# wmtlab/tactileSR

Hardware: AMD Instinct MI355X
Metric: SR samples/sec (4x4->40x40) (higher is better)
Workload: dtype f32 as 2 power-of-two-scaled fp16 planes x 3 MFMA products, fp32 accumulate (fp32-grade); 1 GPU; tactileSR_model eval forward 4x4->40x40, batch=4096/GPU, fp32 in/out (BASELINE configs[1]); batch_per_gpu=4096, scale_factor=10, seqsCnt=1, parallelism=replicas x1, conv_impl=fp16x3, dist_world_size=1

## Files before the change

### tactilesr_amd/csrc/conv_epilogue16.h

```cpp
#pragma once
#include "tsr_common.h"
#include "conv_args.h"
#include "conv_epilogue.h"

template <int COUT, bool EXT, int WN = 2, bool IO16 = false>
__device__ __forceinline__ void conv_epilogue16(const ConvArgs& a, f32x4 (&acc)[4][COUT / (16 * WN)], int ebase, int b0,
                                                int y0, int x0, int wm, int wn, int lane, int HW, float accmul = 1.f) {
  constexpr int NT = COUT / (16 * WN);
  const int cl = lane & 15, ph = lane >> 4;
  const int k4 = cl >> 2, j = cl & 3;
  const int dyl = ph >> 1, dxl = 4 * (ph & 1);
  float amax = 0.f;
  const int b = b0 + wm;
  const bool img_ok = b < a.B;
  const int out_blocks = a.out_ctot >> 4;
  const int res_blocks = a.res_ctot >> 4;
  const int mask_blocks = a.mask_ctot >> 4;
  const int bsafe = img_ok ? b : 0;
  typedef __bf16 ep_bf16x4 __attribute__((ext_vector_type(4)));
  const int gx = x0 + dxl + j;
  const f32x4 one4v = {1.f, 1.f, 1.f, 1.f}, zero4v = {0.f, 0.f, 0.f, 0.f};
  f32x4 pv0[NT], pv1[NT], pv2[NT], pv3[NT], pv4[NT];
  const bool m2 = EXT && a.epi_mode == 2, m0 = !EXT || a.epi_mode == 0;
#pragma unroll
  for (int nt = 0; nt < NT; ++nt) {
    const int nq = wn * (COUT / WN) + nt * 16 + 4 * k4;
    pv0[nt] = one4v; pv1[nt] = zero4v; pv2[nt] = one4v; pv3[nt] = zero4v; pv4[nt] = zero4v;
    if (m0) {
      if (a.scale) pv0[nt] = *(const f32x4*)(a.scale + nq);
      if (a.shift) pv1[nt] = *(const f32x4*)(a.shift + nq);
      if (EXT && a.res_scale) { pv2[nt] = *(const f32x4*)(a.res_scale + nq); pv3[nt] = *(const f32x4*)(a.res_shift + nq); }
    } else if (m2) {
      if (a.scale) pv0[nt] = *(const f32x4*)(a.scale + nq);
      if (a.mask_scale) { pv2[nt] = *(const f32x4*)(a.mask_scale + nq); pv1[nt] = *(const f32x4*)(a.mask_shift + nq); }
      if (a.bn_a) { pv3[nt] = *(const f32x4*)(a.bn_a + nq); pv4[nt] = *(const f32x4*)(a.bn_b + nq); }
    }
  }
#pragma unroll
  for (int nt = 0; nt < NT; ++nt) {
    const int n = wn * (COUT / WN) + nt * 16 + cl;
    const int nq = wn * (COUT / WN) + nt * 16 + 4 * k4;
    const int oq = a.out_coff + nq;
    const size_t oidx4 = (((size_t)bsafe * out_blocks + (oq >> 4)) * HW) * 16 + (oq & 15);
    float* ob4 = a.out + oidx4;
    const float* rb4 = nullptr;
    size_t ridx4 = 0;
    if (a.res) {
      const int rq = a.res_coff + nq;
      ridx4 = (((size_t)bsafe * res_blocks + (rq >> 4)) * HW) * 16 + (rq & 15);
      rb4 = a.res + ridx4;
    }
    if (!EXT || a.epi_mode == 0) {
      const f32x4 sc4 = pv0[nt], sh4 = pv1[nt], rsc4 = pv2[nt], rsh4 = pv3[nt];
      f32x4 rvv[4];
#pragma unroll
      for (int mt = 0; mt < 4; ++mt) {
        const int gy = y0 + 2 * mt + dyl;
        const unsigned pr = (img_ok && gy < a.H && gx < a.W) ? (unsigned)(gy * a.W + gx) * 16u : 0u;
        rvv[mt] = (f32x4){0.f, 0.f, 0.f, 0.f};
        if (rb4) {
          if (IO16) {
            const ep_bf16x4 r16 = *(const ep_bf16x4*)((const __bf16*)a.res + ridx4 + pr);
#pragma unroll
            for (int c = 0; c < 4; ++c) rvv[mt][c] = (float)r16[c];
          } else {
            rvv[mt] = *(const f32x4*)(rb4 + pr);
          }
        }
      }
#pragma unroll
      for (int mt = 0; mt < 4; ++mt) {
        float t0 = acc[mt][nt][0], t1 = acc[mt][nt][1], t2 = acc[mt][nt][2], t3 = acc[mt][nt][3];
        quad_transpose(t0, t1, t2, t3, j);
        const int gy = y0 + 2 * mt + dyl;
        if (img_ok && gy < a.H && gx < a.W) {
          const size_t po = (size_t)(gy * a.W + gx) * 16;
          f32x4 v = {t0, t1, t2, t3};
#pragma unroll
          for (int c = 0; c < 4; ++c) v[c] = (v[c] * accmul) * sc4[c] + sh4[c];
          if (rb4) {
            f32x4 rv = rvv[mt];
            if (EXT && a.res_scale) {
#pragma unroll
              for (int c = 0; c < 4; ++c) rv[c] = tsr_relu(fmaf(rv[c], rsc4[c], rsh4[c]));
            }
#pragma unroll
            for (int c = 0; c < 4; ++c) v[c] += rv[c];
          }
#pragma unroll
          for (int c = 0; c < 4; ++c) {
            if (a.relu) v[c] = tsr_relu(v[c]);
            amax = fmaxf(amax, fabsf(v[c]));
          }
          if (IO16) {
            ep_bf16x4 o16;
#pragma unroll
            for (int c = 0; c < 4; ++c) o16[c] = (__bf16)v[c];
            *(ep_bf16x4*)((__bf16*)a.out + oidx4 + po) = o16;
          } else {
            *(f32x4*)(ob4 + po) = v;
          }
        }
      }
    } else if (EXT && a.epi_mode == 1) {
      float cnt = 0.f, sum = 0.f;
#pragma unroll
      for (int mt = 0; mt < 4; ++mt) {
#pragma unroll
        for (int r = 0; r < 4; ++r) {
          const int gy = y0 + 2 * mt + dyl, gxr = x0 + dxl + r;
          acc[mt][nt][r] *= accmul;
          if (img_ok && gy < a.H && gxr < a.W) {
            const float v = acc[mt][nt][r];
            cnt += 1.f;
            sum += v;
            amax = fmaxf(amax, fabsf(v));
          }
        }
      }
      float mean = cnt > 0.f ? sum / cnt : 0.f;
      float m2 = 0.f;
#pragma unroll
      for (int mt = 0; mt < 4; ++mt) {
#pragma unroll
        for (int r = 0; r < 4; ++r) {
          const int gy = y0 + 2 * mt + dyl, gxr = x0 + dxl + r;
          if (img_ok && gy < a.H && gxr < a.W) {
            const float d = acc[mt][nt][r] - mean;
            m2 = fmaf(d, d, m2);
          }
        }
      }
#pragma unroll
      for (int o = 16; o <= 32; o <<= 1) {
        const float cnt2 = __shfl_xor(cnt, o), mean2 = __shfl_xor(mean, o), m22 = __shfl_xor(m2, o);
        const float tot = cnt + cnt2;
        const float dlt = mean2 - mean;
        const float meanm = tot > 0.f ? mean + dlt * (cnt2 / tot) : 0.f;
        const float m2m = tot > 0.f ? m2 + m22 + dlt * dlt * (cnt * cnt2 / tot) : 0.f;
        cnt = tot; mean = meanm; m2 = m2m;
      }
      if (ph == 0) {
        const size_t e = (size_t)ebase + wm;
        float* sl = a.slab + (e * COUT + n) * 2;
        sl[0] = mean;
        sl[1] = m2;
        if (nt == 0 && cl == 0 && wn == 0) a.slab_cnt[e] = cnt;
      }
#pragma unroll
      for (int mt = 0; mt < 4; ++mt) {
        float t0 = acc[mt][nt][0], t1 = acc[mt][nt][1], t2 = acc[mt][nt][2], t3 = acc[mt][nt][3];
        quad_transpose(t0, t1, t2, t3, j);
        const int gy = y0 + 2 * mt + dyl;
        if (img_ok && gy < a.H && gx < a.W) *(f32x4*)(ob4 + (size_t)(gy * a.W + gx) * 16) = (f32x4){t0, t1, t2, t3};
      }
    } else if (EXT) {
      const int mq = a.mask_coff + nq;
      const float* mb4 = a.mask + (((size_t)bsafe * mask_blocks + (mq >> 4)) * HW) * 16 + (mq & 15);
      const f32x4 zero4 = zero4v;
      const f32x4 sc4 = pv0[nt], msc4 = pv2[nt], msh4 = pv1[nt], ba4 = pv3[nt], bb4 = pv4[nt];
      f32x4 s1 = zero4, s2 = zero4;
      f32x4 mvv[4], rvv[4];
      bool okk[4];
      unsigned pov[4];
#pragma unroll
      for (int mt = 0; mt < 4; ++mt) {
        const int gy = y0 + 2 * mt + dyl;
        okk[mt] = img_ok && gy < a.H && gx < a.W;
        pov[mt] = okk[mt] ? (unsigned)(gy * a.W + gx) * 16u : 0u;
        mvv[mt] = *(const f32x4*)(mb4 + pov[mt]);
        rvv[mt] = rb4 ? *(const f32x4*)(rb4 + pov[mt]) : zero4;
      }
#pragma unroll
      for (int mt = 0; mt < 4; ++mt) {
        float t0 = acc[mt][nt][0], t1 = acc[mt][nt][1], t2 = acc[mt][nt][2], t3 = acc[mt][nt][3];
        quad_transpose(t0, t1, t2, t3, j);
        f32x4 v = {t0, t1, t2, t3};
        const f32x4 mv = okk[mt] ? mvv[mt] : zero4, rv = rvv[mt];
#pragma unroll
        for (int c = 0; c < 4; ++c) {
          float x = (v[c] * accmul) * sc4[c] + rv[c];
          if (!(fmaf(mv[c], msc4[c], msh4[c]) > 0.f)) x = 0.f;
          if (!okk[mt]) x = 0.f;
          v[c] = x;
          amax = fmaxf(amax, fabsf(x));
          s1[c] += x;
// ... 28 lines not shown
```

### tactilesr_amd/csrc/conv_fuse1x1_16.h

```cpp
#pragma once
#include "tsr_common.h"
#include "conv_args.h"
#include "conv_epilogue.h"

typedef _Float16 fq_f16x8 __attribute__((ext_vector_type(8)));
typedef _Float16 fq_f16x4 __attribute__((ext_vector_type(4)));

template <int IMG> struct Fuse1x1Geom16 {
  static constexpr int PIXB = 64;
  static constexpr int ROWB = (8 * 4 + 2) * 16;
  static constexpr int IMGB = 8 * ROWB;
  static constexpr int BLKB = IMG * IMGB;
  static constexpr int BYTES = 8 * BLKB;
};

template <int IMG>
__device__ __forceinline__ void conv_fuse1x1_epilogue16(const ConvArgs& a, f32x4 (&acc)[4][4], char* lds, int b0, int y0,
                                                        int x0, int wm, int wn, int lane, int HW, float accmul) {
  typedef Fuse1x1Geom16<IMG> E;
  const int cl = lane & 15, ph = lane >> 4;
  const int k4 = cl >> 2, j = cl & 3;
  const int dyl = ph >> 1, dxl = 4 * (ph & 1);
  const int b = b0 + wm;
  const bool img_ok = b < a.B;
  const int khalf = ph & 1, bsel = ph >> 1;
  const _Float16* wb = (const _Float16*)a.w2 + ((size_t)(bsel * 2 * 2 + khalf) * 64 + wn * 32 + cl) * 8;
  fq_f16x8 fb[4][2][2];
#pragma unroll
  for (int kk = 0; kk < 4; ++kk)
#pragma unroll
    for (int p = 0; p < 2; ++p)
#pragma unroll
      for (int n2 = 0; n2 < 2; ++n2)
        fb[kk][p][n2] = *(const fq_f16x8*)(wb + (size_t)((2 * kk) * 2 + p) * (2 * 64 * 8) + n2 * 16 * 8);
  const int out_blocks = a.out_ctot >> 4, res_blocks = a.res_ctot >> 4;
  const int bsafe = img_ok ? b : 0;
  const int gx = x0 + dxl + j;
  bool okk[4];
  unsigned pov[4];
  f32x4 rvv[2][4];
#pragma unroll
  for (int mt = 0; mt < 4; ++mt) {
    const int gy = y0 + 2 * mt + dyl;
    okk[mt] = img_ok && gy < a.H && gx < a.W;
    pov[mt] = okk[mt] ? (unsigned)(gy * a.W + gx) * 16u : 0u;
  }
#pragma unroll
  for (int n2 = 0; n2 < 2; ++n2) {
    const int rq = a.res_coff + wn * 32 + n2 * 16 + 4 * k4;
    const float* rb4 = a.res ? a.res + (((size_t)bsafe * res_blocks + (rq >> 4)) * HW) * 16 + (rq & 15) : nullptr;
#pragma unroll
    for (int mt = 0; mt < 4; ++mt) rvv[n2][mt] = rb4 ? *(const f32x4*)(rb4 + pov[mt]) : (f32x4){0.f, 0.f, 0.f, 0.f};
  }
  float bsc[4], bsh[4];
  f32x4 osh[2];
#pragma unroll
  for (int nt = 0; nt < 4; ++nt) {
    const int n = wn * 64 + nt * 16 + cl;
    bsc[nt] = a.scale ? a.scale[n] : 1.f;
    bsh[nt] = a.shift ? a.shift[n] : 0.f;
  }
#pragma unroll
  for (int n2 = 0; n2 < 2; ++n2)
    osh[n2] = a.shift2 ? *(const f32x4*)(a.shift2 + wn * 32 + n2 * 16 + 4 * k4) : (f32x4){0.f, 0.f, 0.f, 0.f};
  float amax = 0.f;
#pragma unroll
  for (int nt = 0; nt < 4; ++nt) {
    const float sc = bsc[nt] * accmul, sh = bsh[nt];
#pragma unroll
    for (int mt = 0; mt < 4; ++mt)
#pragma unroll
      for (int r = 0; r < 4; ++r) {
        const int gy = y0 + 2 * mt + dyl, gx = x0 + dxl + r;
        float v = fmaf(acc[mt][nt][r], sc, sh);
        if (a.relu) v = tsr_relu(v);
        if (!(img_ok && gy < a.H && gx < a.W)) v = 0.f;
        acc[mt][nt][r] = v;
        amax = fmaxf(amax, fabsf(v));
      }
  }
#pragma unroll
  for (int o = 32; o > 0; o >>= 1) amax = fmaxf(amax, __shfl_xor(amax, o));
  float* red = (float*)(lds + E::BYTES);
  if (lane == 0) red[wm * 2 + wn] = amax;
  __syncthreads();
  float tmax = 0.f;
#pragma unroll
  for (int w = 0; w < 2 * IMG; ++w) tmax = fmaxf(tmax, red[w] < 3.0e38f ? red[w] : 0.f);
  float s_e = 1.f;
  if (tmax > 0.f) {
    int e = (int)((__float_as_uint(tmax) >> 23) & 0xFF) - 127;
    int be = 13 - e + 127;
    be = be < 1 ? 1 : (be > 254 ? 254 : be);
    s_e = __uint_as_float((unsigned)be << 23);
  }
#pragma unroll
  for (int nt = 0; nt < 4; ++nt) {
    const int nq = wn * 64 + nt * 16 + 4 * k4;
    char* eb = lds + (nq >> 4) * E::BLKB + wm * E::IMGB + dyl * E::ROWB + (dxl + j) * E::PIXB + (nq & 15) * 2;
#pragma unroll
    for (int mt = 0; mt < 4; ++mt) {
      float t0 = acc[mt][nt][0], t1 = acc[mt][nt][1], t2 = acc[mt][nt][2], t3 = acc[mt][nt][3];
      quad_transpose(t0, t1, t2, t3, j);
      float v[4] = {t0 * s_e, t1 * s_e, t2 * s_e, t3 * s_e};
      fq_f16x4 p0, p1;
#pragma unroll
      for (int c = 0; c < 4; ++c) {
        p0[c] = (_Float16)v[c];
        p1[c] = (_Float16)(v[c] - (float)p0[c]);
      }
      char* dst = eb + (2 * mt) * E::ROWB;
      *(fq_f16x4*)(dst) = p0;
      *(fq_f16x4*)(dst + 32) = p1;
    }
  }
  __syncthreads();
  f32x4 acc2[4][2];
#pragma unroll
  for (int mt = 0; mt < 4; ++mt)
#pragma unroll
    for (int n2 = 0; n2 < 2; ++n2) acc2[mt][n2] = (f32x4){0.f, 0.f, 0.f, 0.f};
  const char* ea = lds + bsel * E::BLKB + wm * E::IMGB + (cl >> 3) * E::ROWB + (cl & 7) * E::PIXB + khalf * 16;
#pragma unroll
  for (int kk = 0; kk < 4; ++kk) {
    fq_f16x8 fa[2][4];
#pragma unroll
    for (int p = 0; p < 2; ++p) {
#pragma unroll
      for (int mt = 0; mt < 4; ++mt) fa[p][mt] = *(const fq_f16x8*)(ea + (2 * kk) * E::BLKB + (2 * mt) * E::ROWB + p * 32);
    }
#pragma unroll
    for (int mt = 0; mt < 4; ++mt)
#pragma unroll
      for (int n2 = 0; n2 < 2; ++n2)
        acc2[mt][n2] = __builtin_amdgcn_mfma_f32_16x16x32_f16(fa[1][mt], fb[kk][0][n2], acc2[mt][n2], 0, 0, 0);
#pragma unroll
    for (int mt = 0; mt < 4; ++mt)
#pragma unroll
      for (int n2 = 0; n2 < 2; ++n2)
        acc2[mt][n2] = __builtin_amdgcn_mfma_f32_16x16x32_f16(fa[0][mt], fb[kk][1][n2], acc2[mt][n2], 0, 0, 0);
#pragma unroll
    for (int mt = 0; mt < 4; ++mt)
#pragma unroll
      for (int n2 = 0; n2 < 2; ++n2)
        acc2[mt][n2] = __builtin_amdgcn_mfma_f32_16x16x32_f16(fa[0][mt], fb[kk][0][n2], acc2[mt][n2], 0, 0, 0);
  }
  const float mul2 = a.w2_inv_scale / s_e;
  float omax = 0.f;
#pragma unroll
  for (int n2 = 0; n2 < 2; ++n2) {
    const int nq2 = wn * 32 + n2 * 16 + 4 * k4;
    const int oq = a.out_coff + nq2;
    const f32x4 sh4 = osh[n2];
    float* ob4 = a.out + (((size_t)bsafe * out_blocks + (oq >> 4)) * HW) * 16 + (oq & 15);
#pragma unroll
    for (int mt = 0; mt < 4; ++mt) {
      float t0 = acc2[mt][n2][0], t1 = acc2[mt][n2][1], t2 = acc2[mt][n2][2], t3 = acc2[mt][n2][3];
      quad_transpose(t0, t1, t2, t3, j);
      if (okk[mt]) {
        f32x4 v = {t0, t1, t2, t3};
        const f32x4 rv = rvv[n2][mt];
#pragma unroll
        for (int c = 0; c < 4; ++c) {
          v[c] = v[c] * mul2 + sh4[c] + rv[c];
          if (a.relu2) v[c] = tsr_relu(v[c]);
          omax = fmaxf(omax, fabsf(v[c]));
        }
        *(f32x4*)(ob4 + pov[mt]) = v;
      }
    }
  }
  if (a.out_amax) {
#pragma unroll
    for (int o = 32; o > 0; o >>= 1) omax = fmaxf(omax, __shfl_xor(omax, o));
    if (lane == 0) publish_amax(a.out_amax, omax);
  }
}
```

### tactilesr_amd/csrc/conv_mfma_k32.hip

```cpp
#include "tsr_common.h"
#include "conv_args.h"
#include "conv_epilogue16.h"
#include "conv_fuse1x1_16.h"
#include "conv_host.h"
#include "tactilesr_hip.h"
#include <type_traits>

typedef _Float16 kf16x8 __attribute__((ext_vector_type(8)));
typedef _Float16 kf16x4 __attribute__((ext_vector_type(4)));

constexpr int k32_row_slots(int px) {
  int rs = px * 4;
  while ((rs & 3) != 2) ++rs;
  return rs;
}

template <int KS, int COUT, int WN, bool DBH = false, int NTHR = 256> struct K32Geom {
  static constexpr int IMG = (NTHR / 64) / WN;
  static constexpr int HH = 8 + KS - 1;
  static constexpr int T = KS * KS;
  static constexpr int HS = (T - 1) / 2;
  static constexpr int PIXB = 64;
  static constexpr int ROWB = k32_row_slots(HH) * 16;
  static constexpr int IMGB = HH * ROWB;
  static constexpr int HALO_B = IMG * IMGB;
  static constexpr int SROWB = k32_row_slots(8) * 16;
  static constexpr int SIMGB = 8 * SROWB;
  static constexpr int SIDE_B = DBH ? 0 : IMG * SIMGB;
  static constexpr int WTAP_B = 2 * 16 * COUT * 2;
  static constexpr int WSLAB_B = 2 * WTAP_B;
  static constexpr int NHB = DBH ? 2 : 1;
  static constexpr int MAIN_LDS = NHB * HALO_B + SIDE_B + 3 * WSLAB_B;
};

constexpr int PAIR_KH[12] = {0, 0, 0, 2, 1, 3, 4, 4, 1, 1, 2, 3};
constexpr int PAIR_KW[12] = {0, 2, 4, 4, 0, 0, 1, 3, 1, 3, 1, 1};
constexpr int PAIR_V[12] = {0, 0, 1, 1, 1, 1, 0, 0, 0, 1, 0, 0};
constexpr int PAIR_OUTER = 8;

template <int KS, int COUT, bool EXT, int WN, bool FUSE2 = false, bool DBH = false, int NTHR = 256, bool PAIR = false>
__global__ __launch_bounds__(NTHR, NTHR == 512 ? 1 : 2) void conv_k32_kernel(const ConvArgs a) {
  static_assert(!PAIR || (KS == 5 && COUT == 128 && !EXT && !FUSE2 && !DBH), "pair form: 5x5 geometry, inference");
  static_assert(COUT == 64 * WN, "every wave owns 64 channels");
  static_assert(!FUSE2 || (!EXT && COUT == 128), "fused 1x1: 128 channels, inference");
  static_assert(NTHR == 256 || (NTHR == 512 && WN == 2), "512 threads: 4 images x 2 C_out halves");
  typedef K32Geom<KS, COUT, WN, DBH, NTHR> G;
  constexpr int NW = NTHR / 64;
  constexpr bool WDMA = !EXT;
  constexpr int IMG = G::IMG, P = KS / 2, HH = G::HH, T = G::T, HS = G::HS, NT = COUT / (16 * WN);
  constexpr int PIXB = G::PIXB, ROWB = G::ROWB, IMGB = G::IMGB, HALO_B = G::HALO_B;
  constexpr int SROWB = G::SROWB, SIMGB = G::SIMGB, SIDE_B = G::SIDE_B;
  constexpr int WTAP_B = G::WTAP_B, WSLAB_B = G::WSLAB_B;
  constexpr int WITEMS = WSLAB_B / 16, WV = (WITEMS + NTHR - 1) / NTHR;
  constexpr int NITEM = IMG * HH * HH * 4, NIT = (NITEM + NTHR - 1) / NTHR;
  constexpr int FUSE_LDS = FUSE2 ? Fuse1x1Geom16<IMG>::BYTES + 64 : 0;
  __shared__ __attribute__((aligned(16))) char lds[G::MAIN_LDS > FUSE_LDS ? G::MAIN_LDS : FUSE_LDS];
  char* halo = lds;
  char* wbuf = lds + G::NHB * HALO_B + SIDE_B;

  const int tid = threadIdx.x;
  const int lane = tid & 63;
  const int wave = tid >> 6;
  const int wave_s = __builtin_amdgcn_readfirstlane(wave);
  const int wm = WN == 2 ? wave >> 1 : wave, wn = WN == 2 ? wave & 1 : 0;
  const int m = lane & 15, g = lane >> 4, khalf = g & 1, tsel = g >> 1;

  float sx = 1.f, accmul = 1.f, sxh = 1.f;
  int bid;
  {
    const int nwg = gridDim.x, q = nwg >> 3, r = nwg & 7;
    const int xcd = blockIdx.x & 7, idx = blockIdx.x >> 3;
    bid = (xcd < r ? xcd * (q + 1) : r * (q + 1) + (xcd - r) * q) + idx;
  }
  const int tpi = a.tiles_x * a.tiles_y;
  const int ig = bid / tpi;
  const int trem = bid - ig * tpi;
  const int ebase = bid * IMG;
  const int ty = trem / a.tiles_x, tx = trem - ty * a.tiles_x;
  const int y0 = ty * 8, x0 = tx * 8, b0 = ig * IMG;
  const int HW = a.H * a.W;
  const int in_blocks = a.in_ctot >> 4;

  int st_src[NIT], st_dst[NIT];
#pragma unroll
  for (int k = 0; k < NIT; ++k) {
    const int it = tid + k * NTHR;
    st_src[k] = -1;
    st_dst[k] = -1;
    if (it < NITEM) {
      const int qd = it & 3, px = it >> 2;
      const int img = px / (HH * HH), rem = px - img * (HH * HH);
      const int hy = rem / HH, hx = rem - hy * HH;
      const int gy = y0 - P + hy, gx = x0 - P + hx, b = b0 + img;
      st_dst[k] = img * IMGB + hy * ROWB + hx * PIXB + qd * 8;
      if (b < a.B && gy >= 0 && gy < a.H && gx >= 0 && gx < a.W)
        st_src[k] = ((img * in_blocks) * HW + gy * a.W + gx) * 16 + qd * 4;
    }
  }
  const float* in_base = a.in + ((size_t)b0 * in_blocks + (a.in_coff >> 4)) * HW * 16;

  const int laneA0 = wm * IMGB + (m >> 3) * ROWB + (m & 7) * PIXB + khalf * 16;
  const int lx = laneA0 + tsel * PIXB;
  constexpr int CK = PAIR ? 3 : KS - 1;
  const int lw = PAIR ? laneA0 + tsel * ROWB
                      : laneA0 + tsel * (ROWB - (KS - 1) * PIXB);
  const int lc = tsel ? laneA0 + CK * ROWB + CK * PIXB
                      : HALO_B + wm * SIMGB + (m >> 3) * SROWB + (m & 7) * PIXB + khalf * 16;
  const int lcs = tsel ? 2 * ROWB : 2 * SROWB;
  const int lcd = laneA0 + (KS - 1) * (ROWB + PIXB) + tsel * HALO_B;
  const int laneB = tsel * WTAP_B + (khalf * COUT + wn * (COUT / WN) + m) * 16;
  const int laneBh = tsel * (WTAP_B / 2) + (khalf * 64 + wn * 32 + m) * 16;

  f32x4 acc[4][NT];
#pragma unroll
  for (int mt = 0; mt < 4; ++mt)
#pragma unroll
    for (int nt = 0; nt < NT; ++nt) acc[mt][nt] = (f32x4){0.f, 0.f, 0.f, 0.f};

  const int nreal = a.cin >> 4;
  const int nchunk = nreal + (nreal & 1);
  const int S = (nchunk >> 1) * T;
  const char* wsrc = (const char*)a.wp;
  const __amdgpu_buffer_rsrc_t wrsrc = __builtin_amdgcn_make_buffer_rsrc((void*)a.wp, 0, 0x7fffffff, 0x00020000);

  f32x4 hsc = {1.f, 1.f, 1.f, 1.f}, hsh = {0.f, 0.f, 0.f, 0.f};
  auto load_halo = [&](int c, f32x4* hv) __attribute__((always_inline)) {
    const float* inc = in_base + (size_t)(c < nreal ? c : nreal - 1) * HW * 16;
    if (EXT && a.in_scale) {
      const int cq = (c < nreal ? c : nreal - 1) * 16 + (tid & 3) * 4;
      hsc = *(const f32x4*)(a.in_scale + cq);
      hsh = *(const f32x4*)(a.in_shift + cq);
    }
#pragma unroll
    for (int k = 0; k < NIT; ++k) hv[k] = *(const f32x4*)(inc + (unsigned)(st_src[k] < 0 ? 0 : st_src[k]));
  };
  auto store_halo = [&](const f32x4* hv, int c, int hb = 0) __attribute__((always_inline)) {
#pragma unroll
    for (int k = 0; k < NIT; ++k) {
      if (st_dst[k] >= 0) {
        f32x4 v = hv[k];
        if (EXT && a.in_scale) {
#pragma unroll
          for (int jj = 0; jj < 4; ++jj) v[jj] = tsr_relu_x2(fmaf(v[jj], hsc[jj], hsh[jj]));
        }
        const bool inside = st_src[k] >= 0 && c < nreal;
#pragma unroll
        for (int jj = 0; jj < 4; ++jj) v[jj] = inside ? v[jj] * sxh : 0.f;
#pragma unroll
        for (int p = 0; p < 2; ++p) {
          kf16x4 bq;
#pragma unroll
          for (int jj = 0; jj < 4; ++jj) {
            bq[jj] = (_Float16)v[jj];
            v[jj] -= (float)bq[jj];
          }
          *(kf16x4*)(halo + hb * HALO_B + st_dst[k] + p * 32) = bq;
        }
      }
    }
  };
#define DMA_BYTES(goff_, slot_, nv_)                                                     \
  {                                                                                      \
    const int vo_ = (int)(goff_) + tid * 16;                                             \
    char* dst_ = wbuf + (slot_) * WSLAB_B + wave_s * 1024;                               \
    _Pragma("unroll") for (int v = 0; v < (nv_); ++v)                                    \
      __builtin_amdgcn_raw_ptr_buffer_load_lds(wrsrc, (__attribute__((address_space(3))) void*)(dst_ + v * NTHR * 16), 16, \
                                               vo_ + v * NTHR * 16, 0, 0, 0);             \
  }
#define LOAD_W(sidx)                                                                     \
  {                                                                                      \
    const f32x4* src_ = (const f32x4*)(wsrc + (size_t)(sidx) * WSLAB_B);                  \
    _Pragma("unroll") for (int v = 0; v < WV; ++v) wreg[v] = src_[tid + v * NTHR];        \
  }
#define STORE_W(slot)                                                                    \
  {                                                                                      \
    char* wb_ = wbuf + (slot) * WSLAB_B;                                                 \
    _Pragma("unroll") for (int v = 0; v < WV; ++v) ((f32x4*)wb_)[tid + v * NTHR] = wreg[v]; \
  }
#define DMA_W(sidx, slot) DMA_BYTES((size_t)(sidx) * WSLAB_B, slot, WV)
#define DMA_WAIT_N(n_) __builtin_amdgcn_s_waitcnt(0x0F70 | ((n_) & 15) | (((n_) >> 4) << 14))
#define DMA_WAIT() DMA_WAIT_N(0)
#define PAIR_HALF(pq_) ((pq_) < 24 && ((pq_) % 12) < PAIR_OUTER)
#define DMA_WP(slot, pq_)                                                                \
  {                                                                                      \
    if (PAIR_HALF(pq_)) { DMA_BYTES(woff, slot, WV / 2); woff += WSLAB_B / 2; }          \
    else { DMA_BYTES(woff, slot, WV); woff += WSLAB_B; }                                 \
  }
#define STEP_BARRIER() __syncthreads()
#define LOAD_A(dst, p_, st_, hb_)                                                        \
  {                                                                                      \
    const int kh_ = PAIR ? PAIR_KH[(st_)] : (2 * (st_)) / KS, kw_ = PAIR ? PAIR_KW[(st_)] : (2 * (st_)) - kh_ * KS; \
    const bool x_ = PAIR ? PAIR_V[(st_)] == 0 : kw_ < KS - 1;                            \
    const char* ab_ = lds + (x_ ? lx : lw) + (hb_) * HALO_B + kh_ * ROWB + kw_ * PIXB + (p_) * 32; \
    _Pragma("unroll") for (int mt = 0; mt < 4; ++mt) dst[mt] = *(const kf16x8*)(ab_ + mt * 2 * ROWB); \
  }
#define LOAD_A_CROSS(dst, p_)                                                            \
  {                                                                                      \
    _Pragma("unroll") for (int mt = 0; mt < 4; ++mt) dst[mt] = *(const kf16x8*)(lds + lc + mt * lcs + (p_) * 32); \
  }
#define LOAD_A_CROSSD(dst, p_)                                                           \
  {                                                                                      \
    _Pragma("unroll") for (int mt = 0; mt < 4; ++mt) dst[mt] = *(const kf16x8*)(lds + lcd + mt * 2 * ROWB + (p_) * 32); \
  }
#define LOAD_B(dst, p_, slot_)                                                           \
  {                                                                                      \
    const char* wb_ = wbuf + (slot_) * WSLAB_B + laneB + (p_) * (2 * COUT * 16);         \
    _Pragma("unroll") for (int nt = 0; nt < NT; ++nt) dst[nt] = *(const kf16x8*)(wb_ + nt * 256); \
  }
#define LOAD_B_HI(dst, p_, slot_)                                                        \
  {                                                                                      \
    const char* wb_ = wbuf + (slot_) * WSLAB_B + laneBh + (p_) * (2 * 64 * 16);          \
    _Pragma("unroll") for (int nt = 2; nt < NT; ++nt) dst[nt] = *(const kf16x8*)(wb_ + (nt - 2) * 256); \
  }
#define MFMA_PHASE_HI(A_, B_)                                                            \
  _Pragma("unroll") for (int mt = 0; mt < 4; ++mt)                                       \
    _Pragma("unroll") for (int nt = 2; nt < NT; ++nt)                                    \
      acc[mt][nt] = __builtin_amdgcn_mfma_f32_16x16x32_f16(A_[mt], B_[nt], acc[mt][nt], 0, 0, 0);
#define MFMA_PHASE(A_, B_)                                                               \
  _Pragma("unroll") for (int mt = 0; mt < 4; ++mt)                                       \
    _Pragma("unroll") for (int nt = 0; nt < NT; ++nt)                                    \
      acc[mt][nt] = __builtin_amdgcn_mfma_f32_16x16x32_f16(A_[mt], B_[nt], acc[mt][nt], 0, 0, 0);
#define INTERLEAVE(n_, per_)                                                             \
  _Pragma("unroll") for (int i_ = 0; i_ < (n_); ++i_) {                                  \
    __builtin_amdgcn_sched_group_barrier(0x008, (per_), 0);                              \
    __builtin_amdgcn_sched_group_barrier(0x100, 1, 0);                                   \
  }

  auto operand_scales = [&]() __attribute__((always_inline)) {
    float mx = a.in_amax ? *a.in_amax : 0.f;
    if (EXT && a.in_scale) {
      __shared__ float bnd[2 * NW];
      float ms = 0.f, mt = 0.f;
      for (int c = threadIdx.x; c < a.cin; c += NTHR) {
        ms = fmaxf(ms, fabsf(a.in_scale[c]));
        mt = fmaxf(mt, fabsf(a.in_shift[c]));
      }
#pragma unroll
      for (int o = 32; o > 0; o >>= 1) {
        ms = fmaxf(ms, __shfl_xor(ms, o));
        mt = fmaxf(mt, __shfl_xor(mt, o));
      }
      if (lane == 0) { bnd[wave * 2] = ms; bnd[wave * 2 + 1] = mt; }
      __syncthreads();
      ms = 0.f; mt = 0.f;
#pragma unroll
      for (int w = 0; w < NW; ++w) { ms = fmaxf(ms, bnd[2 * w]); mt = fmaxf(mt, bnd[2 * w + 1]); }
      mx = mx * ms + mt;
    }
    if (mx > 0.f) {
      int e = (int)((__float_as_uint(mx) >> 23) & 0xFF) - 127;
      int be = 13 - e + 127;
      be = be < 1 ? 1 : (be > 254 ? 254 : be);
      sx = __uint_as_float((unsigned)be << 23);
    }
    float w_inv = a.w_inv_scale;
    if (a.w_amax) {
      const float wmx = *a.w_amax;
      w_inv = 1.f;
      if (wmx > 0.f && wmx < 3.0e38f) {
        int be = 127 - (13 - ((int)((__float_as_uint(wmx) >> 23) & 0xFF) - 127));
        be = be < 1 ? 1 : (be > 254 ? 254 : be);
        w_inv = __uint_as_float((unsigned)be << 23);
      }
    }
    accmul = w_inv / sx;
    sxh = (EXT && a.in_scale) ? 0.5f * sx : sx;
  };

  f32x4 hv[NIT], wreg[WDMA ? 1 : WV];
  size_t woff = 0;
  load_halo(0, hv);
  if constexpr (PAIR) {
    DMA_WP(0, 0);
    DMA_WP(1, 1);
    operand_scales();
  } else if constexpr (WDMA) {
    DMA_W(0, 0);
    if (S > 1) DMA_W(1, 1);
    operand_scales();
  } else {
    LOAD_W(0);
    operand_scales();
    STORE_W(0);
    if (S > 1) { LOAD_W(1); STORE_W(1); }
  }
  store_halo(hv, 0);
  if constexpr (WDMA) { DMA_WAIT(); } else { if (S > 2) LOAD_W(2); }
  __syncthreads();

  kf16x8 A0[4], A1[4], B0[NT] = {}, B1[NT] = {};
  LOAD_A(A1, 1, 0, 0);
  if constexpr (PAIR) { LOAD_B_HI(B0, 0, 0); } else { LOAD_B(B0, 0, 0); }

  constexpr int SCI = IMG * 256 / NTHR, SCS = NTHR / 256;
  const int sc_t = tid & 255, sc_i0 = tid >> 8;
  const int sc_src = sc_i0 * IMGB + ((sc_t >> 5) + CK) * ROWB + (((sc_t >> 2) & 7) + CK) * PIXB + (sc_t & 3) * 16;
  const int sc_dst = HALO_B + sc_i0 * SIMGB + (sc_t >> 5) * SROWB + ((sc_t >> 2) & 7) * PIXB + (sc_t & 3) * 16;

  int s = 0;
  int slot = 0;
  auto block = [&](int c, auto oddc) __attribute__((always_inline)) {
    constexpr int ODD = decltype(oddc)::value;
    constexpr int NST = HS + ODD;
#pragma unroll
    for (int st = 0; st < NST; ++st) {
      const int slot1 = slot == 2 ? 0 : slot + 1;
      const int slot2 = slot1 == 2 ? 0 : slot1 + 1;
      const bool cross = ODD && st == HS;
      f32x4 sidev[SCI];
      if (WDMA && s + 2 < S) {
        if constexpr (PAIR) { DMA_WP(slot2, (ODD * HS + st + 2) % 25); } else { DMA_W(s + 2, slot2); }
      }
      const bool outer = PAIR && st < PAIR_OUTER;
      const bool next_outer = PAIR && (st + 1 < PAIR_OUTER || st + 1 == NST);
      if (cross) { LOAD_A_CROSS(A0, 0); } else { LOAD_A(A0, 0, st, 0); }
      if (outer) { LOAD_B_HI(B1, 1, slot); } else { LOAD_B(B1, 1, slot); }
      if (!ODD && st == 0) {
#pragma unroll
        for (int k = 0; k < SCI; ++k) sidev[k] = *(const f32x4*)(lds + sc_src + k * SCS * IMGB);
      }
      if (st == NST - 2 && c + 1 < nchunk) load_halo(c + 1, hv);
      if (outer) {
        MFMA_PHASE_HI(A1, B0);
        if (!ODD && st == 0) { INTERLEAVE(6 + SCI, 1); } else { INTERLEAVE(6, 1); }
      } else {
        MFMA_PHASE(A1, B0);
        if (!ODD && st == 0) { INTERLEAVE(8 + SCI, 1); } else { INTERLEAVE(8, 2); }
      }
      if (st + 1 < NST) {
        if (ODD && st + 1 == HS) { LOAD_A_CROSS(A1, 1); } else { LOAD_A(A1, 1, st + 1, 0); }
      }
      if (outer) {
        MFMA_PHASE_HI(A0, B0);
        if (st + 1 < NST) { INTERLEAVE(4, 2); }
      } else {
        MFMA_PHASE(A0, B0);
        if (st + 1 < NST) { INTERLEAVE(4, 4); }
      }
      if (next_outer) { LOAD_B_HI(B0, 0, slot1); } else { LOAD_B(B0, 0, slot1); }
      if (outer) {
        MFMA_PHASE_HI(A0, B1);
        if (next_outer) { INTERLEAVE(2, 4); } else { INTERLEAVE(4, 2); }
      } else {
        MFMA_PHASE(A0, B1);
        if (next_outer) { INTERLEAVE(2, 8); } else { INTERLEAVE(4, 4); }
      }
      if (!ODD && st == 0) {
#pragma unroll
        for (int k = 0; k < SCI; ++k) *(f32x4*)(lds + sc_dst + k * SCS * SIMGB) = sidev[k];
      }
      if constexpr (WDMA) {
        if (st == NST - 2 && c + 1 < nchunk) { DMA_WAIT_N(NIT); } else { DMA_WAIT(); }
      } else {
        if (s + 2 < S) STORE_W(slot2);
        if (s + 3 < S) LOAD_W(s + 3);
      }
      STEP_BARRIER();
      if (st + 1 == NST && c + 1 < nchunk) {
        store_halo(hv, c + 1);
        __syncthreads();
        LOAD_A(A1, 1, 0, 0);
      }
      ++s;
      slot = slot1;
    }
  };
  if constexpr (!DBH) {
    for (int c = 0; c < nchunk; c += 2) {
      block(c, std::integral_constant<int, 0>());
      block(c + 1, std::integral_constant<int, 1>());
    }
  } else {
    for (int c = 0; c < nchunk; c += 2) {
#pragma unroll
      for (int p = 0; p < T; ++p) {
        const int slot1 = slot == 2 ? 0 : slot + 1;
        const int slot2 = slot1 == 2 ? 0 : slot1 + 1;
        if (WDMA && s + 2 < S) DMA_W(s + 2, slot2);
        if (p == HS) { LOAD_A_CROSSD(A0, 0); }
        else if (p < HS) { LOAD_A(A0, 0, p, 0); }
        else { LOAD_A(A0, 0, p - HS - 1, 1); }
        LOAD_B(B1, 1, slot);
        if (p == 0) load_halo(c + 1, hv);
        if (p == HS + 1 && c + 2 < nchunk) load_halo(c + 2, hv);
        MFMA_PHASE(A1, B0);
        INTERLEAVE(8, 2);
        if (p + 1 == HS) { LOAD_A_CROSSD(A1, 1); }
        else if (p + 1 < HS) { LOAD_A(A1, 1, p + 1, 0); }
        else if (p + 1 < T) { LOAD_A(A1, 1, p - HS, 1); }
        else { LOAD_A(A1, 1, 0, 0); }
        MFMA_PHASE(A0, B0);
        INTERLEAVE(4, 4);
        LOAD_B(B0, 0, slot1);
        MFMA_PHASE(A0, B1);
        INTERLEAVE(4, 4);
        if (p == HS - 2) store_halo(hv, c + 1, 1);
        if (p == T - 2 && c + 2 < nchunk) store_halo(hv, c + 2, 0);
        if constexpr (WDMA) {
          if (p == 0 || (p == HS + 1 && c + 2 < nchunk)) { DMA_WAIT_N(NIT); } else { DMA_WAIT(); }
        } else {
          if (s + 2 < S) STORE_W(slot2);
          if (s + 3 < S) LOAD_W(s + 3);
        }
        STEP_BARRIER();
        ++s;
        slot = slot1;
      }
    }
  }
#undef DMA_W
#undef LOAD_W
#undef STORE_W
#undef DMA_WP
#undef DMA_BYTES
#undef DMA_WAIT
#undef DMA_WAIT_N
#undef PAIR_HALF
#undef STEP_BARRIER
#undef LOAD_A
#undef LOAD_A_CROSS
#undef LOAD_A_CROSSD
#undef LOAD_B
#undef LOAD_B_HI
#undef MFMA_PHASE_HI
#undef MFMA_PHASE
#undef INTERLEAVE

  if constexpr (FUSE2) conv_fuse1x1_epilogue16<IMG>(a, acc, lds, b0, y0, x0, wm, wn, lane, HW, accmul);
  else conv_epilogue16<COUT, EXT, WN>(a, acc, ebase, b0, y0, x0, wm, wn, lane, HW, accmul);
}

int tsr_conv_k32_images(int cout) { (void)cout; return 4; }

template <int KS, int COUT, bool EXT>
static int launch_k32(const ConvArgs& a, hipStream_t st) {
  constexpr int WN = COUT / 64;
  if constexpr (COUT == 128 && EXT) {
    const int grid = ((a.B + 3) / 4) * a.tiles_x * a.tiles_y;
    hipLaunchKernelGGL((conv_k32_kernel<KS, COUT, EXT, WN, false, KS == 3, 512>), dim3(grid), dim3(512), 0, st, a);
    return tsr_check_launch();
  }
  constexpr int IMG = 4 / WN;
  const int grid = ((a.B + IMG - 1) / IMG) * a.tiles_x * a.tiles_y;
  hipLaunchKernelGGL((conv_k32_kernel<KS, COUT, EXT, WN, false, KS == 3>), dim3(grid), dim3(256), 0, st, a);
  return tsr_check_launch();
}

template <bool EXT> static int dispatch_k32(const ConvArgs& a, int cout, int ks, hipStream_t st) {
  return for_cout_ks(cout, ks, [&](auto CO, auto KS) {
    if constexpr (decltype(KS)::value > 1) return launch_k32<decltype(KS)::value, decltype(CO)::value, EXT>(a, st);
    else return (int)TSR_ERR_ARG;
  });
}
int tsr_conv_k32(const ConvArgs& a, int cout, int ks, bool ext, hipStream_t st) {
  return ext ? dispatch_k32<true>(a, cout, ks, st) : dispatch_k32<false>(a, cout, ks, st);
}

__host__ __device__ inline int pair_logical_channel(int k) {
  const int wn = k >> 6, nt = (k >> 4) & 3, c = k & 15;
  return (nt < 2 ? 0 : 64) + wn * 32 + (nt & 1) * 16 + c;
}
extern "C" int tsr_pair_channel_perm(int* perm128) {
  if (!perm128) return TSR_ERR_ARG;
  for (int k = 0; k < 128; ++k) perm128[k] = pair_logical_channel(k);
  return TSR_OK;
}

__global__ void pack_pair_kernel(const float* __restrict__ w3, const float* __restrict__ w5, _Float16* __restrict__ wp,
                                 int cin, float wscale, const float* __restrict__ w_amax) {
  if (w_amax) {
    const float wm = *w_amax;
    wscale = 1.f;
    if (wm > 0.f && wm < 3.0e38f) {
      int be = 127 + 13 - ((int)((__float_as_uint(wm) >> 23) & 0xFF) - 127);
      be = be < 1 ? 1 : (be > 254 ? 254 : be);
      wscale = __uint_as_float((unsigned)be << 23);
    }
  }
  const int cin_p = (cin + 31) & ~31;
  const size_t total = (size_t)128 * cin_p * 25;
  for (size_t i = blockIdx.x * (size_t)blockDim.x + threadIdx.x; i < total; i += (size_t)gridDim.x * blockDim.x) {
    const int j = i & 7;
    size_t r = i >> 3;
    const int k = r & 127; r >>= 7;
    const int kh2 = r & 1; r >>= 1;
    const int tap = r % 25;
    const int chunk = r / 25;
    const int ci = chunk * 16 + kh2 * 8 + j;
    const int kh = tap / 5, kw = tap - kh * 5;
    const int nt = (k >> 4) & 3, ch = (k >> 6) * 32 + (nt & 1) * 16 + (k & 15);
    float v = 0.f;
    if (ci < cin) {
      if (nt >= 2) v = w5[((size_t)ch * cin + ci) * 25 + tap];
      else if (kh >= 1 && kh <= 3 && kw >= 1 && kw <= 3) v = w3[((size_t)ch * cin + ci) * 9 + (kh - 1) * 3 + (kw - 1)];
    }
    v *= wscale;
    int pos = 24;
#pragma unroll
    for (int st = 0; st < 12; ++st) {
      if (kh == PAIR_KH[st] && kw == PAIR_KW[st]) pos = 2 * st;
      if (kh == PAIR_KH[st] + PAIR_V[st] && kw == PAIR_KW[st] + 1 - PAIR_V[st]) pos = 2 * st + 1;
    }
    const int odd = chunk & 1;
    const bool half = pos < 2 * PAIR_OUTER;
    if (half && nt < 2) continue;
    size_t base = (size_t)(chunk >> 1) * (2 * 65536 + 8192);
    if (pos >= 24) base += 2 * 65536 + (size_t)odd * 4096;
    else if (half) base += (size_t)odd * 65536 + (size_t)(pos >> 1) * 4096 + (size_t)(pos & 1) * 2048;
    else base += (size_t)odd * 65536 + 32768 + (size_t)((pos - 16) >> 1) * 8192 + (size_t)(pos & 1) * 4096;
    const int nch = half ? 64 : 128;
    const int kk = half ? (k >> 6) * 32 + (nt - 2) * 16 + (k & 15) : k;
    for (int p = 0; p < 2; ++p) {
// ... 39 lines not shown
```

Before: 31840 samples/s.

## Specialize full-tile epilogues, use fma_mix fp16 splitting, and raise MFMA loop priority

```diff
diff --git a/tactilesr_amd/csrc/conv_epilogue16.h b/tactilesr_amd/csrc/conv_epilogue16.h
--- a/tactilesr_amd/csrc/conv_epilogue16.h
+++ b/tactilesr_amd/csrc/conv_epilogue16.h
@@ -2,10 +2,12 @@
 #include "tsr_common.h"
 #include "conv_args.h"
 #include "conv_epilogue.h"
+#include <type_traits>
 
 template <int COUT, bool EXT, int WN = 2, bool IO16 = false>
 __device__ __forceinline__ void conv_epilogue16(const ConvArgs& a, f32x4 (&acc)[4][COUT / (16 * WN)], int ebase, int b0,
-                                                int y0, int x0, int wm, int wn, int lane, int HW, float accmul = 1.f) {
+                                                int y0, int x0, int wm, int wn, int lane, int HW, float accmul = 1.f,
+                                                bool full = false) {
   constexpr int NT = COUT / (16 * WN);
   const int cl = lane & 15, ph = lane >> 4;
   const int k4 = cl >> 2, j = cl & 3;
@@ -51,57 +53,62 @@
       rb4 = a.res + ridx4;
     }
     if (!EXT || a.epi_mode == 0) {
-      const f32x4 sc4 = pv0[nt], sh4 = pv1[nt], rsc4 = pv2[nt], rsh4 = pv3[nt];
-      f32x4 rvv[4];
-#pragma unroll
-      for (int mt = 0; mt < 4; ++mt) {
-        const int gy = y0 + 2 * mt + dyl;
-        const unsigned pr = (img_ok && gy < a.H && gx < a.W) ? (unsigned)(gy * a.W + gx) * 16u : 0u;
-        rvv[mt] = (f32x4){0.f, 0.f, 0.f, 0.f};
-        if (rb4) {
-          if (IO16) {
-            const ep_bf16x4 r16 = *(const ep_bf16x4*)((const __bf16*)a.res + ridx4 + pr);
-#pragma unroll
-            for (int c = 0; c < 4; ++c) rvv[mt][c] = (float)r16[c];
-          } else {
-            rvv[mt] = *(const f32x4*)(rb4 + pr);
-          }
-        }
-      }
-#pragma unroll
-      for (int mt = 0; mt < 4; ++mt) {
-        float t0 = acc[mt][nt][0], t1 = acc[mt][nt][1], t2 = acc[mt][nt][2], t3 = acc[mt][nt][3];
-        quad_transpose(t0, t1, t2, t3, j);
-        const int gy = y0 + 2 * mt + dyl;
-        if (img_ok && gy < a.H && gx < a.W) {
-          const size_t po = (size_t)(gy * a.W + gx) * 16;
-          f32x4 v = {t0, t1, t2, t3};
-#pragma unroll
-          for (int c = 0; c < 4; ++c) v[c] = (v[c] * accmul) * sc4[c] + sh4[c];
+      auto mode0 = [&](auto fullc) __attribute__((always_inline)) {
+        constexpr bool FULL = decltype(fullc)::value;
+        const f32x4 sc4 = pv0[nt], sh4 = pv1[nt], rsc4 = pv2[nt], rsh4 = pv3[nt];
+        f32x4 rvv[4];
+#pragma unroll
+        for (int mt = 0; mt < 4; ++mt) {
+          const int gy = y0 + 2 * mt + dyl;
+          const bool ok = FULL | (img_ok & (gy < a.H) & (gx < a.W));
+          const unsigned pr = ok ? (unsigned)(gy * a.W + gx) * 16u : 0u;
+          rvv[mt] = (f32x4){0.f, 0.f, 0.f, 0.f};
           if (rb4) {
-            f32x4 rv = rvv[mt];
-            if (EXT && a.res_scale) {
-#pragma unroll
-              for (int c = 0; c < 4; ++c) rv[c] = tsr_relu(fmaf(rv[c], rsc4[c], rsh4[c]));
-            }
-#pragma unroll
-            for (int c = 0; c < 4; ++c) v[c] += rv[c];
-          }
-#pragma unroll
-          for (int c = 0; c < 4; ++c) {
-            if (a.relu) v[c] = tsr_relu(v[c]);
-            amax = fmaxf(amax, fabsf(v[c]));
-          }
-          if (IO16) {
-            ep_bf16x4 o16;
-#pragma unroll
-            for (int c = 0; c < 4; ++c) o16[c] = (__bf16)v[c];
-            *(ep_bf16x4*)((__bf16*)a.out + oidx4 + po) = o16;
-          } else {
-            *(f32x4*)(ob4 + po) = v;
-          }
-        }
-      }
+            if (IO16) {
+              const ep_bf16x4 r16 = *(const ep_bf16x4*)((const __bf16*)a.res + ridx4 + pr);
+#pragma unroll
+              for (int c = 0; c < 4; ++c) rvv[mt][c] = (float)r16[c];
+            } else {
+              rvv[mt] = *(const f32x4*)(rb4 + pr);
+            }
+          }
+        }
+#pragma unroll
+        for (int mt = 0; mt < 4; ++mt) {
+          float t0 = acc[mt][nt][0], t1 = acc[mt][nt][1], t2 = acc[mt][nt][2], t3 = acc[mt][nt][3];
+          quad_transpose(t0, t1, t2, t3, j);
+          const int gy = y0 + 2 * mt + dyl;
+          if (FULL || (img_ok && gy < a.H && gx < a.W)) {
+            const size_t po = (size_t)(gy * a.W + gx) * 16;
+            f32x4 v = {t0, t1, t2, t3};
+#pragma unroll
+            for (int c = 0; c < 4; ++c) v[c] = (v[c] * accmul) * sc4[c] + sh4[c];
+            if (rb4) {
+              f32x4 rv = rvv[mt];
+              if (EXT && a.res_scale) {
+#pragma unroll
+                for (int c = 0; c < 4; ++c) rv[c] = tsr_relu(fmaf(rv[c], rsc4[c], rsh4[c]));
+              }
+#pragma unroll
+              for (int c = 0; c < 4; ++c) v[c] += rv[c];
+            }
+#pragma unroll
+            for (int c = 0; c < 4; ++c) {
+              if (a.relu) v[c] = tsr_relu(v[c]);
+              amax = fmaxf(amax, fabsf(v[c]));
+            }
+            if (IO16) {
+              ep_bf16x4 o16;
+#pragma unroll
+              for (int c = 0; c < 4; ++c) o16[c] = (__bf16)v[c];
+              *(ep_bf16x4*)((__bf16*)a.out + oidx4 + po) = o16;
+            } else {
+              *(f32x4*)(ob4 + po) = v;
+            }
+          }
+        }
+      };
+      if (!EXT && full) mode0(std::true_type()); else mode0(std::false_type());
     } else if (EXT && a.epi_mode == 1) {
       float cnt = 0.f, sum = 0.f;
 #pragma unroll
diff --git a/tactilesr_amd/csrc/conv_fuse1x1_16.h b/tactilesr_amd/csrc/conv_fuse1x1_16.h
--- a/tactilesr_amd/csrc/conv_fuse1x1_16.h
+++ b/tactilesr_amd/csrc/conv_fuse1x1_16.h
@@ -2,9 +2,28 @@
 #include "tsr_common.h"
 #include "conv_args.h"
 #include "conv_epilogue.h"
+#include <type_traits>
 
 typedef _Float16 fq_f16x8 __attribute__((ext_vector_type(8)));
 typedef _Float16 fq_f16x4 __attribute__((ext_vector_type(4)));
+
+template <bool SREG> __device__ __forceinline__ void k32_split_planes(const f32x4 x, float s, fq_f16x4& h1, fq_f16x4& h2) {
+  unsigned a[2], b[2];
+#define K32_SPLIT(SC_)                                                                                                     \
+  asm("v_fma_mixlo_f16 %0, %1, %2, 0" : "=v"(a[0]) : "v"(x[0]), SC_(s));                                                    \
+  asm("v_fma_mixlo_f16 %0, %1, %2, 0" : "=v"(a[1]) : "v"(x[2]), SC_(s));                                                    \
+  asm("v_fma_mixhi_f16 %0, %1, %2, 0" : "+v"(a[0]) : "v"(x[1]), SC_(s));                                                    \
+  asm("v_fma_mixhi_f16 %0, %1, %2, 0" : "+v"(a[1]) : "v"(x[3]), SC_(s));                                                    \
+  asm("v_fma_mixlo_f16 %0, %1, %2, -%3 op_sel_hi:[0,0,1]" : "=v"(b[0]) : "v"(x[0]), SC_(s), "v"(a[0]));                     \
+  asm("v_fma_mixlo_f16 %0, %1, %2, -%3 op_sel_hi:[0,0,1]" : "=v"(b[1]) : "v"(x[2]), SC_(s), "v"(a[1]));                     \
+  asm("v_fma_mixhi_f16 %0, %1, %2, -%3 op_sel:[0,0,1] op_sel_hi:[0,0,1]" : "+v"(b[0]) : "v"(x[1]), SC_(s), "v"(a[0]));      \
+  asm("v_fma_mixhi_f16 %0, %1, %2, -%3 op_sel:[0,0,1] op_sel_hi:[0,0,1]" : "+v"(b[1]) : "v"(x[3]), SC_(s), "v"(a[1]));
+  if constexpr (SREG) { K32_SPLIT("s") } else { K32_SPLIT("v") }
+#undef K32_SPLIT
+  typedef unsigned u32x2 __attribute__((ext_vector_type(2)));
+  h1 = __builtin_bit_cast(fq_f16x4, (u32x2){a[0], a[1]});
+  h2 = __builtin_bit_cast(fq_f16x4, (u32x2){b[0], b[1]});
+}
 
 template <int IMG> struct Fuse1x1Geom16 {
   static constexpr int PIXB = 64;
@@ -16,7 +35,8 @@
 
 template <int IMG>
 __device__ __forceinline__ void conv_fuse1x1_epilogue16(const ConvArgs& a, f32x4 (&acc)[4][4], char* lds, int b0, int y0,
-                                                        int x0, int wm, int wn, int lane, int HW, float accmul) {
+                                                        int x0, int wm, int wn, int lane, int HW, float accmul,
+                                                        bool full = false) {
   typedef Fuse1x1Geom16<IMG> E;
   const int cl = lane & 15, ph = lane >> 4;
   const int k4 = cl >> 2, j = cl & 3;
@@ -26,13 +46,16 @@
   const int khalf = ph & 1, bsel = ph >> 1;
   const _Float16* wb = (const _Float16*)a.w2 + ((size_t)(bsel * 2 * 2 + khalf) * 64 + wn * 32 + cl) * 8;
   fq_f16x8 fb[4][2][2];
-#pragma unroll
-  for (int kk = 0; kk < 4; ++kk)
-#pragma unroll
-    for (int p = 0; p < 2; ++p)
-#pragma unroll
-      for (int n2 = 0; n2 < 2; ++n2)
-        fb[kk][p][n2] = *(const fq_f16x8*)(wb + (size_t)((2 * kk) * 2 + p) * (2 * 64 * 8) + n2 * 16 * 8);
+  auto load_fb = [&](int kk0) __attribute__((always_inline)) {
+#pragma unroll
+    for (int kk = kk0; kk < kk0 + 2; ++kk)
+#pragma unroll
+      for (int p = 0; p < 2; ++p)
+#pragma unroll
+        for (int n2 = 0; n2 < 2; ++n2)
+          fb[kk][p][n2] = *(const fq_f16x8*)(wb + (size_t)((2 * kk) * 2 + p) * (2 * 64 * 8) + n2 * 16 * 8);
+  };
+  load_fb(0);
   const int out_blocks = a.out_ctot >> 4, res_blocks = a.res_ctot >> 4;
   const int bsafe = img_ok ? b : 0;
   const int gx = x0 + dxl + j;
@@ -42,7 +65,7 @@
 #pragma unroll
   for (int mt = 0; mt < 4; ++mt) {
     const int gy = y0 + 2 * mt + dyl;
-    okk[mt] = img_ok && gy < a.H && gx < a.W;
+    okk[mt] = full || (img_ok && gy < a.H && gx < a.W);
     pov[mt] = okk[mt] ? (unsigned)(gy * a.W + gx) * 16u : 0u;
   }
 #pragma unroll
@@ -64,21 +87,24 @@
   for (int n2 = 0; n2 < 2; ++n2)
     osh[n2] = a.shift2 ? *(const f32x4*)(a.shift2 + wn * 32 + n2 * 16 + 4 * k4) : (f32x4){0.f, 0.f, 0.f, 0.f};
   float amax = 0.f;
-#pragma unroll
-  for (int nt = 0; nt < 4; ++nt) {
-    const float sc = bsc[nt] * accmul, sh = bsh[nt];
-#pragma unroll
-    for (int mt = 0; mt < 4; ++mt)
-#pragma unroll
-      for (int r = 0; r < 4; ++r) {
-        const int gy = y0 + 2 * mt + dyl, gx = x0 + dxl + r;
-        float v = fmaf(acc[mt][nt][r], sc, sh);
-        if (a.relu) v = tsr_relu(v);
-        if (!(img_ok && gy < a.H && gx < a.W)) v = 0.f;
-        acc[mt][nt][r] = v;
-        amax = fmaxf(amax, fabsf(v));
-      }
-  }
+  auto bn_relu = [&](auto fullc) __attribute__((always_inline)) {
+#pragma unroll
+    for (int nt = 0; nt < 4; ++nt) {
+      const float sc = bsc[nt] * accmul, sh = bsh[nt];
+#pragma unroll
+      for (int mt = 0; mt < 4; ++mt)
+#pragma unroll
+        for (int r = 0; r < 4; ++r) {
+          const int gy = y0 + 2 * mt + dyl, gx = x0 + dxl + r;
+          float v = fmaf(acc[mt][nt][r], sc, sh);
+          if (a.relu) v = tsr_relu(v);
+          if constexpr (!decltype(fullc)::value) v = (img_ok & (gy < a.H) & (gx < a.W)) ? v : 0.f;
+          acc[mt][nt][r] = v;
+          amax = fmaxf(amax, fabsf(v));
+        }
+    }
+  };
+  if (full) bn_relu(std::true_type()); else bn_relu(std::false_type());
 #pragma unroll
   for (int o = 32; o > 0; o >>= 1) amax = fmaxf(amax, __shfl_xor(amax, o));
   float* red = (float*)(lds + E::BYTES);
@@ -102,13 +128,8 @@
     for (int mt = 0; mt < 4; ++mt) {
       float t0 = acc[mt][nt][0], t1 = acc[mt][nt][1], t2 = acc[mt][nt][2], t3 = acc[mt][nt][3];
       quad_transpose(t0, t1, t2, t3, j);
-      float v[4] = {t0 * s_e, t1 * s_e, t2 * s_e, t3 * s_e};
       fq_f16x4 p0, p1;
-#pragma unroll
-      for (int c = 0; c < 4; ++c) {
-        p0[c] = (_Float16)v[c];
-        p1[c] = (_Float16)(v[c] - (float)p0[c]);
-      }
+      k32_split_planes<false>((f32x4){t0, t1, t2, t3}, s_e, p0, p1);
       char* dst = eb + (2 * mt) * E::ROWB;
       *(fq_f16x4*)(dst) = p0;
       *(fq_f16x4*)(dst + 32) = p1;
@@ -123,6 +144,7 @@
   const char* ea = lds + bsel * E::BLKB + wm * E::IMGB + (cl >> 3) * E::ROWB + (cl & 7) * E::PIXB + khalf * 16;
 #pragma unroll
   for (int kk = 0; kk < 4; ++kk) {
+    if (kk == 0) load_fb(2);
     fq_f16x8 fa[2][4];
 #pragma unroll
     for (int p = 0; p < 2; ++p) {
@@ -147,29 +169,33 @@
   }
   const float mul2 = a.w2_inv_scale / s_e;
   float omax = 0.f;
-#pragma unroll
-  for (int n2 = 0; n2 < 2; ++n2) {
-    const int nq2 = wn * 32 + n2 * 16 + 4 * k4;
-    const int oq = a.out_coff + nq2;
-    const f32x4 sh4 = osh[n2];
-    float* ob4 = a.out + (((size_t)bsafe * out_blocks + (oq >> 4)) * HW) * 16 + (oq & 15);
-#pragma unroll
-    for (int mt = 0; mt < 4; ++mt) {
-      float t0 = acc2[mt][n2][0], t1 = acc2[mt][n2][1], t2 = acc2[mt][n2][2], t3 = acc2[mt][n2][3];
-      quad_transpose(t0, t1, t2, t3, j);
-      if (okk[mt]) {
-        f32x4 v = {t0, t1, t2, t3};
-        const f32x4 rv = rvv[n2][mt];
-#pragma unroll
-        for (int c = 0; c < 4; ++c) {
-          v[c] = v[c] * mul2 + sh4[c] + rv[c];
-          if (a.relu2) v[c] = tsr_relu(v[c]);
-          omax = fmaxf(omax, fabsf(v[c]));
+  auto out_stage = [&](auto fullc) __attribute__((always_inline)) {
+#pragma unroll
+    for (int n2 = 0; n2 < 2; ++n2) {
+      const int nq2 = wn * 32 + n2 * 16 + 4 * k4;
+      const int oq = a.out_coff + nq2;
+      const f32x4 sh4 = osh[n2];
+      float* ob4 = a.out + (((size_t)bsafe * out_blocks + (oq >> 4)) * HW) * 16 + (oq & 15);
+#pragma unroll
+      for (int mt = 0; mt < 4; ++mt) {
+        float t0 = acc2[mt][n2][0], t1 = acc2[mt][n2][1], t2 = acc2[mt][n2][2], t3 = acc2[mt][n2][3];
+        quad_transpose(t0, t1, t2, t3, j);
+        if (decltype(fullc)::value || okk[mt]) {
+          f32x4 v = {t0, t1, t2, t3};
+          const f32x4 rv = rvv[n2][mt];
+#pragma unroll
+          for (int c = 0; c < 4; ++c) {
+            v[c] = v[c] * mul2 + sh4[c] + rv[c];
+            asm("" : "+v"(v[c]));
+            if (a.relu2) v[c] = tsr_relu(v[c]);
+            omax = fmaxf(omax, fabsf(v[c]));
+          }
+          *(f32x4*)(ob4 + pov[mt]) = v;
         }
-        *(f32x4*)(ob4 + pov[mt]) = v;
       }
     }
-  }
+  };
+  if (full) out_stage(std::true_type()); else out_stage(std::false_type());
   if (a.out_amax) {
 #pragma unroll
     for (int o = 32; o > 0; o >>= 1) omax = fmaxf(omax, __shfl_xor(omax, o));
diff --git a/tactilesr_amd/csrc/conv_mfma_k32.hip b/tactilesr_amd/csrc/conv_mfma_k32.hip
--- a/tactilesr_amd/csrc/conv_mfma_k32.hip
+++ b/tactilesr_amd/csrc/conv_mfma_k32.hip
@@ -80,6 +80,8 @@
   const int y0 = ty * 8, x0 = tx * 8, b0 = ig * IMG;
   const int HW = a.H * a.W;
   const int in_blocks = a.in_ctot >> 4;
+  const bool tile_full = !EXT && b0 + IMG <= a.B && y0 + 8 <= a.H && x0 + 8 <= a.W;
+  const bool halo_in = tile_full && y0 >= P && y0 + 8 + P <= a.H && x0 >= P && x0 + 8 + P <= a.W;
 
   int st_src[NIT], st_dst[NIT];
 #pragma unroll
@@ -134,7 +136,29 @@
 #pragma unroll
     for (int k = 0; k < NIT; ++k) hv[k] = *(const f32x4*)(inc + (unsigned)(st_src[k] < 0 ? 0 : st_src[k]));
   };
+  auto store_halo_inf = [&](const f32x4* hv, int hb, bool block_real, auto insidec) __attribute__((always_inline)) {
+#pragma unroll
+    for (int k = 0; k < NIT; ++k) {
+      if (st_dst[k] >= 0) {
+        f32x4 v = hv[k];
+        if constexpr (!decltype(insidec)::value) {
+          const bool inside = st_src[k] >= 0 && block_real;
+#pragma unroll
+          for (int jj = 0; jj < 4; ++jj) v[jj] = inside ? v[jj] : 0.f;
+        }
+        kf16x4 h1, h2;
+        k32_split_planes<true>(v, sxh, h1, h2);
+        *(kf16x4*)(halo + hb * HALO_B + st_dst[k]) = h1;
+        *(kf16x4*)(halo + hb * HALO_B + st_dst[k] + 32) = h2;
+      }
+    }
+  };
   auto store_halo = [&](const f32x4* hv, int c, int hb = 0) __attribute__((always_inline)) {
+    if constexpr (!EXT) {
+      if (halo_in && c < nreal) store_halo_inf(hv, hb, true, std::true_type());
+      else store_halo_inf(hv, hb, c < nreal, std::false_type());
+      return;
+    }
 #pragma unroll
     for (int k = 0; k < NIT; ++k) {
       if (st_dst[k] >= 0) {
@@ -297,6 +321,7 @@
   const int sc_src = sc_i0 * IMGB + ((sc_t >> 5) + CK) * ROWB + (((sc_t >> 2) & 7) + CK) * PIXB + (sc_t & 3) * 16;
   const int sc_dst = HALO_B + sc_i0 * SIMGB + (sc_t >> 5) * SROWB + ((sc_t >> 2) & 7) * PIXB + (sc_t & 3) * 16;
 
+  constexpr bool LOOP_PRIO = !EXT;
   int s = 0;
   int slot = 0;
   auto block = [&](int c, auto oddc) __attribute__((always_inline)) {
@@ -356,6 +381,7 @@
         if (s + 3 < S) LOAD_W(s + 3);
       }
       STEP_BARRIER();
+      if (LOOP_PRIO && !ODD && st == 0 && c == 0) __builtin_amdgcn_s_setprio(1);
       if (st + 1 == NST && c + 1 < nchunk) {
         store_halo(hv, c + 1);
         __syncthreads();
@@ -403,11 +429,13 @@
           if (s + 3 < S) LOAD_W(s + 3);
         }
         STEP_BARRIER();
+        if (LOOP_PRIO && p == 0 && c == 0) __builtin_amdgcn_s_setprio(1);
         ++s;
         slot = slot1;
       }
     }
   }
+  if (LOOP_PRIO) __builtin_amdgcn_s_setprio(0);
 #undef DMA_W
 #undef LOAD_W
 #undef STORE_W
@@ -426,8 +454,8 @@
 #undef MFMA_PHASE
 #undef INTERLEAVE
 
-  if constexpr (FUSE2) conv_fuse1x1_epilogue16<IMG>(a, acc, lds, b0, y0, x0, wm, wn, lane, HW, accmul);
-  else conv_epilogue16<COUT, EXT, WN>(a, acc, ebase, b0, y0, x0, wm, wn, lane, HW, accmul);
+  if constexpr (FUSE2) conv_fuse1x1_epilogue16<IMG>(a, acc, lds, b0, y0, x0, wm, wn, lane, HW, accmul, tile_full);
+  else conv_epilogue16<COUT, EXT, WN>(a, acc, ebase, b0, y0, x0, wm, wn, lane, HW, accmul, tile_full);
 }
 
 int tsr_conv_k32_images(int cout) { (void)cout; return 4; }
```

New measurement: 32120 samples/s (median of 6 runs). No clear change (+0.9%).
